# Xharlie/pointnerf

Hardware: AMD Instinct MI355X
Metric: rays/sec (render+bwd) NeRF-synth lego 800^2, K=8, 128 samp/ray (higher is better)
Workload: dtype f32 in / out / accumulate; forward GEMM operands as 2 x f16 planes (22-bit) on the f16 MFMA, 3 products per multiply-add; input-gradient GEMMs: f16 leading product + e4m3 cross terms (csrc/mixq.h), 2 product equivalents; weight-gradient GEMM operands as one f16 plane each

## Files before the change

pointnerf_amd/csrc/aggregate.hip:

```cpp
#include "mixq.h"
#include <stdlib.h>

extern "C" int pnerf_mlp_layout(int feat_dim, int64_t *offsets) {
    if (feat_dim != PN_F || !offsets) return PNERF_E_UNSUP;
    const int64_t o[PNERF_MLP_NTENSORS + 1] = {PO_W1, PO_B1, PO_W2, PO_B2, PO_W3, PO_B3, PO_W4, PO_B4, PO_W5, PO_B5,
                                               PO_WC1, PO_BC1, PO_WC2, PO_BC2, PO_WC3, PO_BC3, PO_WC4, PO_BC4, PO_TOTAL};
    for (int i = 0; i <= PNERF_MLP_NTENSORS; ++i) offsets[i] = o[i];
    return 0;
}
extern "C" size_t pnerf_mlp_packed_bytes(void) { return (size_t)PKC_END; }

namespace {
struct PackHDesc { int src, ld, trans, Mreal, Kreal, NCH, MB, dst, cm1, ck1; };
__device__ __forceinline__ float pn_pack_scale(const char *packed, int cm1, int ck1, int m, int k) {
    float f = 1.f;
    if (cm1 && m < (cm1 - 1 < PN_CS_C1 ? PN_H : PN_HC)) f = pn_col_scale(packed, cm1 - 1)[m];
    if (ck1) f *= pn_col_scale_inv(packed, ck1 - 1)[k];
    return f;
}
struct ColScaleDesc { int first, units, n_cons; struct { int src, ld, rows; } cons[2]; };
struct ColScaleTable { ColScaleDesc d[7]; };
__global__ __launch_bounds__(256) void k_pack_colscale(ColScaleTable t, const float *__restrict__ params, char *__restrict__ packed) {
    __shared__ unsigned red[256];
    const ColScaleDesc d = t.d[blockIdx.x];
// ... 48 lines not shown
    pn_mode_saturate();
    const PackMDesc d = t.d[blockIdx.y];
    auto W = [&](int m, int k) -> float {
        return (m < d.Mreal && k < d.Kreal) ? (d.trans ? params[d.src + k * d.ld + m] * pn_pack_scale(packed, d.cm1, d.ck1, m, k) : params[d.src + m * d.ld + k]) : 0.f;
    };
    uint4 *img = reinterpret_cast<uint4 *>(packed + d.dst);
    unsigned *sc = reinterpret_cast<unsigned *>(img + PN_MIMG_U4(d.NT, d.MB));
    const int nsup = PN_MIX_NS * d.MB * 64, ntail = d.NT * d.MB * 64;
    for (int e = blockIdx.x * 256 + threadIdx.x; e < nsup + ntail; e += gridDim.x * 256) {
        if (e < nsup) {
            const int lane = e & 63, mb = (e >> 6) % d.MB, s = (e >> 6) / d.MB, m = 32 * mb + (lane & 31), hf = lane >> 5;
            uint4 *o = img + ((size_t)(s * d.MB + mb) * 8) * 64 + lane;
#pragma unroll
            for (int r = 0; r < 4; ++r) {
                const int k0 = 64 * s + 16 * r + 8 * hf;
                unsigned h[4], lo[4];
#pragma unroll
                for (int j = 0; j < 4; ++j) pn_split2_rne(W(m, k0 + 2 * j), W(m, k0 + 2 * j + 1), h[j], lo[j]);
                o[r * 64] = make_uint4(h[0], h[1], h[2], h[3]);
            }
            unsigned scw = 0u;
#pragma unroll
            for (int j = 0; j < 2; ++j) {
                float wh[16], wm[16], mx = 0.f;
#pragma unroll
                for (int i = 0; i < 32; ++i) {
                    const float w = W(m, 64 * s + 32 * j + i);
#ifdef PN_EMU
                    const float wc = fmaxf(fminf(w, 65504.f), -65504.f);
#else
                    const float wc = w;
#endif
                    const float h = (float)(_Float16)wc;
                    mx = fmaxf(mx, fmaxf(fabsf(h), fabsf(w - h) * 2048.f));
                }
#pragma unroll
                for (int i = 0; i < 16; ++i) {
                    const float w = W(m, 8 * (8 * s + 4 * j + 2 * hf + (i >> 3)) + (i & 7));
#ifdef PN_EMU
                    const float wc = fmaxf(fminf(w, 65504.f), -65504.f);
#else
                    const float wc = w;
#endif
                    wh[i] = (float)(_Float16)wc; wm[i] = w - wh[i];
                }
                int ex = 0;
                const float fr = frexpf(mx, &ex);
                int be = mx > 0.f ? (fr > 0.875f ? ex - 8 : ex - 9) : 0;
                be = be < -100 ? -100 : (be > 100 ? 100 : be);
                const float sh = __uint_as_float((unsigned)(be + 127) << 23), sm = __uint_as_float((unsigned)(be + 127 - 11) << 23);
                scw |= (unsigned)(be + 127) << (8 * j);
#pragma unroll
                for (int tt = 0; tt < 2; ++tt) {
                    unsigned q[4];
#pragma unroll
                    for (int w4 = 0; w4 < 4; ++w4) {
                        const float *src = (w4 < 2 ? wm : wh) + 8 * tt + 4 * (w4 & 1);
                        const float scl = w4 < 2 ? sm : sh;
                        pn_s2 r = {0, 0};
                        r = __builtin_amdgcn_cvt_scalef32_pk_fp8_f32(r, src[0], src[1], scl, false);
                        r = __builtin_amdgcn_cvt_scalef32_pk_fp8_f32(r, src[2], src[3], scl, true);
                        q[w4] = __builtin_bit_cast(unsigned, r);
                    }
                    o[(4 + 2 * j + tt) * 64] = make_uint4(q[0], q[1], q[2], q[3]);
                }
            }
            sc[(size_t)(s * d.MB + mb) * 64 + lane] = scw;
        } else {
            const int e2 = e - nsup, lane = e2 & 63, mb = (e2 >> 6) % d.MB, tc = (e2 >> 6) / d.MB, m = 32 * mb + (lane & 31);
            const int k0 = 256 + 16 * tc + 8 * (lane >> 5);
            unsigned h[4], lo[4];
#pragma unroll
            for (int j = 0; j < 4; ++j) pn_split2_sat(W(m, k0 + 2 * j), W(m, k0 + 2 * j + 1), h[j], lo[j]);
            uint4 *o = img + (size_t)PN_MIX_NS * d.MB * 8 * 64 + ((size_t)(tc * d.MB + mb) * 2) * 64 + lane;
            o[0] = make_uint4(h[0], h[1], h[2], h[3]);
            o[64] = make_uint4(lo[0], lo[1], lo[2], lo[3]);
        }
    }
}
}

extern "C" int pnerf_mlp_pack(const float *d_params, void *d_packed, void *stream) {
    if (!d_params || !d_packed) return PNERF_E_INVAL;
    PackHTable th = {{
        {PO_W1, PN_IN1, 0, PN_H, PN_IN1, 18, 8, PKH_F1},
        {PO_W2, PN_H, 0, PN_H, PN_H, 16, 8, PKH_F2},
        {PO_W3, PN_IN3, 0, PN_H, PN_IN3, 17, 8, PKH_F3},
        {PO_W4, PN_H, 0, PN_H, PN_H, 16, 8, PKH_F4},
        {PO_W4, PN_H, 1, PN_H, PN_H, 16, 8, PKH_D4, PN_CS_L3 + 1, PN_CS_L4 + 1},
        {PO_W3, PN_IN3, 1, PN_IN3, PN_H, 16, 9, PKH_D3, PN_CS_L2 + 1, PN_CS_L3 + 1},
        {PO_W2, PN_H, 1, PN_H, PN_H, 16, 8, PKH_D2, PN_CS_L1 + 1, PN_CS_L2 + 1},
        {PO_W1, PN_IN1, 1, 32 * PN_MB_D1, PN_H, 16, PN_MB_D1, PKH_D1, 0, PN_CS_L1 + 1},
        {PO_WC1, PN_INC, 0, PN_HC, PN_INC, 18, 4, PKH_FC1},
        {PO_WC2, PN_HC, 0, PN_HC, PN_HC, 8, 4, PKH_FC2},
        {PO_WC3, PN_HC, 0, PN_HC, PN_HC, 8, 4, PKH_FC3},
        {PO_WC3, PN_HC, 1, PN_HC, PN_HC, 8, 4, PKH_DC3, PN_CS_C2 + 1, PN_CS_C3 + 1},
        {PO_WC2, PN_HC, 1, PN_HC, PN_HC, 8, 4, PKH_DC2, PN_CS_C1 + 1, PN_CS_C2 + 1},
        {PO_WC1, PN_INC, 1, PN_H, PN_HC, 8, 8, PKH_DC1, PN_CS_L4 + 1, PN_CS_C1 + 1},
        {PO_W1 + 32 * PN_MB_D1, PN_IN1, 1, PN_IN1 - 32 * PN_MB_D1, PN_H, 16, 2, PKH_D1T, 0, PN_CS_L1 + 1},
    }};
    const ColScaleTable tc = {{
        {PN_CS_L1, PN_H, 1, {{PO_W2, PN_H, PN_H}}},
        {PN_CS_L2, PN_H, 1, {{PO_W3, PN_IN3, PN_H}}},
        {PN_CS_L3, PN_H, 1, {{PO_W4, PN_H, PN_H}}},
        {PN_CS_L4, PN_H, 2, {{PO_W5, PN_H, 1}, {PO_WC1, PN_INC, PN_HC}}},
        {PN_CS_C1, PN_HC, 1, {{PO_WC2, PN_HC, PN_HC}}},
        {PN_CS_C2, PN_HC, 1, {{PO_WC3, PN_HC, PN_HC}}},
        {PN_CS_C3, PN_HC, 1, {{PO_WC4, PN_HC, 3}}},
    }};
    PnProfScope prof(PNK_PACK, (hipStream_t)stream);
    hipLaunchKernelGGL(k_pack_colscale, dim3(7), dim3(256), 0, (hipStream_t)stream, tc, d_params, (char *)d_packed);
    hipLaunchKernelGGL(k_pack_h, dim3(40, 15), dim3(256), 0, (hipStream_t)stream, th, d_params, (char *)d_packed);
    PackMTable tm = {{
        {PO_W1, PN_IN1, 0, PN_H, PN_IN1, 2, 8, PKM_F1},
        {PO_W2, PN_H, 0, PN_H, PN_H, 0, 8, PKM_F2},
        {PO_W3, PN_IN3, 0, PN_H, PN_IN3, 1, 8, PKM_F3},
        {PO_W4, PN_H, 0, PN_H, PN_H, 0, 8, PKM_F4},
        {PO_W4, PN_H, 1, PN_H, PN_H, 0, 8, PKM_D4, PN_CS_L3 + 1, PN_CS_L4 + 1},
        {PO_W3, PN_IN3, 1, PN_IN3, PN_H, 0, 9, PKM_D3, PN_CS_L2 + 1, PN_CS_L3 + 1},
        {PO_W2, PN_H, 1, PN_H, PN_H, 0, 8, PKM_D2, PN_CS_L1 + 1, PN_CS_L2 + 1},
        {PO_W1, PN_IN1, 1, 32 * PN_MB_D1, PN_H, 0, PN_MB_D1, PKM_D1, 0, PN_CS_L1 + 1},
        {PO_W1 + 32 * PN_MB_D1, PN_IN1, 1, PN_IN1 - 32 * PN_MB_D1, PN_H, 0, 2, PKM_D1T, 0, PN_CS_L1 + 1},
    }};
    hipLaunchKernelGGL(k_pack_mix, dim3(12, 9), dim3(256), 0, (hipStream_t)stream, tm, d_params, (char *)d_packed);
    PN_CHECK_LAUNCH();
    return 0;
}

namespace {
template <int NT>
__global__ __launch_bounds__(256) void k_debug_mix_gemm(const float *__restrict__ x, const char *__restrict__ img, float *__restrict__ out) {
    extern __shared__ __attribute__((aligned(16))) char smem_d[];
    pn_mode_saturate();
    constexpr int K = 256 + 16 * NT;
    char *X = smem_d;
    const int tid = threadIdx.x, lane = tid & 63, wave = __builtin_amdgcn_readfirstlane(tid >> 6);
    for (int e = tid; e < PN_TILE * (K / 4); e += 256) {
        const int row = e / (K / 4), col = 4 * (e % (K / 4));
        const float4 v = *reinterpret_cast<const float4 *>(x + row * K + col);
        if (col < 256) pn_xq_store4(X, row, col, v.x, v.y, v.z, v.w);
        else pn_xt_store4(X, row, col, v.x, v.y, v.z, v.w);
    }
    __syncthreads();
    f32x16 acc[2][2];
    pn_acc_zero(acc);
    pn_gemm_mix<PN_MIX_NS, NT, 8, 2>(X, img, 2 * wave, lane, acc);
#pragma unroll
    for (int fb = 0; fb < 2; ++fb)
#pragma unroll
        for (int rb = 0; rb < 2; ++rb)
#pragma unroll
            for (int g = 0; g < 4; ++g)
#pragma unroll
                for (int i = 0; i < 4; ++i) out[(32 * rb + (lane & 31)) * PN_H + pn_d_feat(2 * wave + fb, g, lane) + i] = acc[fb][rb][4 * g + i];
}
}

extern "C" int pnerf_debug_mix_gemm(const float *d_w, int K, const float *d_x, void *d_img, float *d_out, void *stream) {
    if (!d_w || !d_x || !d_img || !d_out || (K != 256 && K != 272 && K != 288)) return PNERF_E_INVAL;
    hipStream_t s = (hipStream_t)stream;
    const int NT = (K - 256) / 16;
    PackMTable tm = {{{0, K, 0, PN_H, K, NT, 8, 0}}};
    hipLaunchKernelGGL(k_pack_mix, dim3(12, 1), dim3(256), 0, s, tm, d_w, (char *)d_img);
    const void *fn = NT == 0 ? (const void *)k_debug_mix_gemm<0> : NT == 1 ? (const void *)k_debug_mix_gemm<1> : (const void *)k_debug_mix_gemm<2>;
    if (hipFuncSetAttribute(fn, hipFuncAttributeMaxDynamicSharedMemorySize, PN_XBYTES) != hipSuccess) return PNERF_E_LAUNCH;
    if (NT == 0) hipLaunchKernelGGL(k_debug_mix_gemm<0>, dim3(1), dim3(256), PN_XBYTES, s, d_x, (const char *)d_img, d_out);
    else if (NT == 1) hipLaunchKernelGGL(k_debug_mix_gemm<1>, dim3(1), dim3(256), PN_XBYTES, s, d_x, (const char *)d_img, d_out);
    else hipLaunchKernelGGL(k_debug_mix_gemm<2>, dim3(1), dim3(256), PN_XBYTES, s, d_x, (const char *)d_img, d_out);
    PN_CHECK_LAUNCH();
    return 0;
}

namespace {
__global__ __launch_bounds__(64) void k_debug_mfma_f16(const uint4 *__restrict__ a, const uint4 *__restrict__ b, float *__restrict__ d) {
    f32x16 acc;
#pragma unroll
    for (int r = 0; r < 16; ++r) acc[r] = 0.f;
    acc = __builtin_amdgcn_mfma_f32_32x32x16_f16(__builtin_bit_cast(pn_h8, a[threadIdx.x]), __builtin_bit_cast(pn_h8, b[threadIdx.x]), acc, 0, 0, 0);
#pragma unroll
    for (int r = 0; r < 16; ++r) d[threadIdx.x * 16 + r] = acc[r];
}
}
namespace {
__global__ __launch_bounds__(256) void k_debug_split(const float *__restrict__ x, long long n, unsigned *__restrict__ h, unsigned *__restrict__ m, int sat) {
    for (long long i = (long long)blockIdx.x * 256 + threadIdx.x; 2 * i < n; i += (long long)gridDim.x * 256) {
        unsigned hh, mm;
        if (sat) pn_split2_sat(x[2 * i], x[2 * i + 1], hh, mm);
        else pn_split2(x[2 * i], x[2 * i + 1], hh, mm);
        h[i] = hh; m[i] = mm;
    }
}
}
extern "C" int pnerf_debug_split(const float *d_x, int64_t n, void *d_h, void *d_m, int sat, void *stream) {
    if (!d_x || !d_h || !d_m || n < 0 || (n & 1)) return PNERF_E_INVAL;
    if (n == 0) return 0;
    hipLaunchKernelGGL(k_debug_split, dim3(64), dim3(256), 0, (hipStream_t)stream, d_x, (long long)n, (unsigned *)d_h, (unsigned *)d_m, sat);
    PN_CHECK_LAUNCH();
    return 0;
}

namespace {
template <int NF> __global__ __launch_bounds__(256) void k_debug_pe(const float *__restrict__ x, long long n, float *__restrict__ out) {
    for (long long i = (long long)blockIdx.x * 256 + threadIdx.x; i < n; i += (long long)gridDim.x * 256) {
        float s[NF], c[NF];
        pn_pe_octaves<NF>(x[i], s, c);
#pragma unroll
        for (int f = 0; f < NF; ++f) { out[(i * NF + f) * 2] = s[f]; out[(i * NF + f) * 2 + 1] = c[f]; }
    }
}
}
extern "C" int pnerf_debug_pe(const float *d_x, int64_t n, int nfreq, float *d_out, void *stream) {
    if (!d_x || !d_out || n < 0 || nfreq < 1 || nfreq > 5) return PNERF_E_INVAL;
    if (n == 0) return 0;
    hipStream_t s = (hipStream_t)stream;
    switch (nfreq) {
        case 1: hipLaunchKernelGGL(k_debug_pe<1>, dim3(64), dim3(256), 0, s, d_x, (long long)n, d_out); break;
        case 2: hipLaunchKernelGGL(k_debug_pe<2>, dim3(64), dim3(256), 0, s, d_x, (long long)n, d_out); break;
        case 3: hipLaunchKernelGGL(k_debug_pe<3>, dim3(64), dim3(256), 0, s, d_x, (long long)n, d_out); break;
        case 4: hipLaunchKernelGGL(k_debug_pe<4>, dim3(64), dim3(256), 0, s, d_x, (long long)n, d_out); break;
        default: hipLaunchKernelGGL(k_debug_pe<5>, dim3(64), dim3(256), 0, s, d_x, (long long)n, d_out); break;
    }
    PN_CHECK_LAUNCH();
    return 0;
}

extern "C" int pnerf_debug_mfma_f16(const void *d_a, const void *d_b, float *d_out, void *stream) {
    if (!d_a || !d_b || !d_out) return PNERF_E_INVAL;
    hipLaunchKernelGGL(k_debug_mfma_f16, dim3(1), dim3(64), 0, (hipStream_t)stream, (const uint4 *)d_a, (const uint4 *)d_b, d_out);
    PN_CHECK_LAUNCH();
    return 0;
}

size_t pn_saved_walk(void *base, long long n_valid, int K, PnSaved &s) {
    const int TS = pn_tile_samples(K);
    const long long tiles = (n_valid + TS - 1) / TS + 2 * PN_NCLS + 1;
    s.rows = tiles * PN_TILE;
    s.samples = ((tiles * TS + PN_CTILE - 1) / PN_CTILE + 1) * PN_CTILE;
    PnCarver cv(base);
    const size_t rg = (size_t)s.rows / 8, rgc = (size_t)s.samples / 8;
    auto planes = [&](uint4 *&x0, uint4 *&h2, uint4 *&h1, uint4 *&h3, uint4 *&dy1, uint4 *&dy2, uint4 *&dy3, uint4 *&dy4) {
        x0 = cv.take<uint4>(rg * PN_NF1); h2 = cv.take<uint4>(rg * PN_NF1);
        h1 = cv.take<uint4>(rg * PN_H); h3 = cv.take<uint4>(rg * PN_H);
        dy1 = cv.take<uint4>(rg * PN_H); dy2 = cv.take<uint4>(rg * PN_H);
        dy3 = cv.take<uint4>(rg * PN_H); dy4 = cv.take<uint4>(rg * PN_H);
    };
    auto cplanes = [&](uint4 *&xc, uint4 *&c1, uint4 *&c2, uint4 *&dc1, uint4 *&dc2, uint4 *&dc3) {
        xc = cv.take<uint4>(rgc * PN_NF1); c1 = cv.take<uint4>(rgc * PN_HC); c2 = cv.take<uint4>(rgc * PN_HC);
        dc1 = cv.take<uint4>(rgc * PN_HC); dc2 = cv.take<uint4>(rgc * PN_HC); dc3 = cv.take<uint4>(rgc * PN_HC);
    };
    planes(s.x0k, s.h2k, s.h1k, s.h3k, s.dy1k, s.dy2k, s.dy3k, s.dy4k);
    s.h4r = cv.take<uint4>((size_t)s.rows * 32 * 2);
    s.arow = cv.take<float>((size_t)s.rows); s.rmeta = cv.take<int4>((size_t)s.rows);
    s.lmask = cv.take<unsigned>((size_t)tiles * 3 * 512);
    s.gscale = cv.take<unsigned>(PN_GS_WORDS);
    s.fs = cv.take<float>((size_t)s.samples * PN_H); s.dfs = cv.take<float>((size_t)s.samples * PN_H);
    s.c3 = cv.take<float>((size_t)s.samples * PN_HC);
    cplanes(s.xck, s.c1k, s.c2k, s.dc1k, s.dc2k, s.dc3k);
    s.cmask = cv.take<unsigned>((size_t)s.samples / PN_CTILE * 2 * 256);
    s.wg2 = pn_arith().wgrad_planes == 2 ? 1 : 0;
    s.x0m = s.h1m = s.h2m = s.h3m = s.dy1m = s.dy2m = s.dy3m = s.dy4m = nullptr;
    s.xcm = s.c1m = s.c2m = s.dc1m = s.dc2m = s.dc3m = nullptr;
    if (s.wg2) {
        planes(s.x0m, s.h2m, s.h1m, s.h3m, s.dy1m, s.dy2m, s.dy3m, s.dy4m);
        cplanes(s.xcm, s.c1m, s.c2m, s.dc1m, s.dc2m, s.dc3m);
    }
    pn_cls_walk(cv, s);
    return cv.off;
}
void pn_cls_walk(PnCarver &cv, PnSaved &s) {
    s.cls_list = cv.take<int>((size_t)s.samples);
    s.cls_info = cv.take<int>(PN_CI_WORDS);
    s.cls_tmp = cv.take<int>((size_t)2 * s.samples + pn_scan_scratch_ints(s.samples) + 8);
}
size_t pn_saved_bytes(long long n_valid, int K) { PnSaved s; return pn_saved_walk(nullptr, n_valid, K, s); }
PnSaved pn_saved_carve(void *base, long long n_valid, int K) { PnSaved s; pn_saved_walk(base, n_valid, K, s); return s; }

extern "C" size_t pnerf_agg_saved_bytes(int64_t n_valid_samples, int K) {
    if (K <= 0 || K > PNERF_MAX_K || n_valid_samples < 0) return 0;
    return pn_saved_bytes(n_valid_samples, K);
}

namespace {
struct FwdArgs {
    pnerf_camera cam;
    const float *xyz, *emb, *conf, *dir, *color;
    const float *params;
    const float4 *packed;
    const float *raydir, *sample_loc;
    const float *xyz_pers, *loc_pers;
    const int *pidx, *valid_list, *counters;
    const int *cls_list, *cls_info;
    int cls, Kstride;
    int save_x0;
    int R, SR, K, TS;
    long long cap_samples;
    float *decoded, *weight;
    PnSaved sv;
};
struct FwdArgsF : FwdArgs { const float *frames; };
template <bool FRAMES> struct FwdArgsOf { using type = FwdArgs; };
template <> struct FwdArgsOf<true> { using type = FwdArgsF; };

namespace {
struct ClsArgs { const int *valid_list, *counters, *pidx; int K, n, ncls; int kc[PN_NCLS], ts[PN_NCLS]; };

__global__ void k_cls_flags(ClsArgs c, int which, int *__restrict__ flags) {
    const int vs = blockIdx.x * blockDim.x + threadIdx.x;
    if (vs >= c.n) return;
    const int Ns = c.counters[0] < c.n ? c.counters[0] : c.n;
    int f = 0;
    if (vs < Ns) {
        const long long si = c.valid_list[vs];
        int hv = 0;
        for (int k = 0; k < c.K; ++k)
            if (c.pidx[si * c.K + k] >= 0) hv = k + 1;
        int cl = 0;
        for (int j = 1; j < c.ncls; ++j)
            if (hv <= c.kc[j]) cl = j;
        f = cl == which;
    }
    flags[vs] = f;
}

__global__ void k_cls_gather(ClsArgs c, int which, const int *__restrict__ pos, const int *__restrict__ count, int *__restrict__ cls_list,
                             int *__restrict__ info) {
    const int n = *count, base = info[PN_CI_VBASE + which];
    for (int i = blockIdx.x * blockDim.x + threadIdx.x; i < n; i += gridDim.x * blockDim.x) cls_list[base + i] = c.valid_list[pos[i]];
    if (blockIdx.x == 0 && threadIdx.x == 0) {
        const int tiles = (n + c.ts[which] - 1) / c.ts[which], tb = info[PN_CI_TBASE + which];
        info[PN_CI_COUNT + which] = n;
        if (which + 1 < PN_NCLS) { info[PN_CI_VBASE + which + 1] = base + n; info[PN_CI_TBASE + which + 1] = tb + tiles + 1; }
        info[PN_CI_TILES] = tb + tiles + 1;
    }
}

__global__ void k_cls_zero_gaps(PnSaved sv, int ncls, int save_x0) {
    const int c = blockIdx.y;
    if (c >= ncls) return;
    if ((blockIdx.x == 0 && !save_x0) || (blockIdx.x == 8 && save_x0)) return;
    const long long gap = (c + 1 < PN_NCLS ? sv.cls_info[PN_CI_TBASE + c + 1] : sv.cls_info[PN_CI_TILES]) - 1;
    uint4 *arrs[9] = {sv.x0k, sv.h2k, sv.h1k, sv.h3k, sv.dy1k, sv.dy2k, sv.dy3k, sv.dy4k, sv.x0k};
    uint4 *arrm[9] = {sv.x0m, sv.h2m, sv.h1m, sv.h3m, sv.dy1m, sv.dy2m, sv.dy3m, sv.dy4m, nullptr};
    const int which = blockIdx.x;
    const int nf = which == 8 ? 64 : which < 2 ? PN_NF1 : PN_H;
    uint4 *p = arrs[which] + gap * 8 * nf;
    for (int i = threadIdx.x; i < 8 * nf; i += blockDim.x) p[i] = make_uint4(0u, 0u, 0u, 0u);
    if (sv.wg2 && arrm[which]) {
        uint4 *pm = arrm[which] + gap * 8 * nf;
        for (int i = threadIdx.x; i < 8 * nf; i += blockDim.x) pm[i] = make_uint4(0u, 0u, 0u, 0u);
    }
}
}

}

int pn_class_slots(int K, int kc[PN_NCLS]) {
    if (K % 4 == 0) { kc[0] = K; kc[1] = K / 2; kc[2] = K / 4; return 3; }
    kc[0] = K; kc[1] = kc[2] = 0;
    return 1;
}

int pn_classify(const PnSaved &sv, const int32_t *d_valid_list, const int32_t *d_counters, const int32_t *d_pidx, int K, long long n_valid,
                bool train, bool save_x0, hipStream_t s) {
    ClsArgs c;
    c.valid_list = d_valid_list; c.counters = d_counters; c.pidx = d_pidx; c.K = K; c.n = (int)n_valid;
    c.ncls = pn_class_slots(K, c.kc);
    for (int j = 0; j < PN_NCLS; ++j) c.ts[j] = c.kc[j] > 0 ? pn_tile_samples(c.kc[j]) : 1;
    if (hipMemsetAsync(sv.cls_info, 0, PN_CI_WORDS * sizeof(int), s) != hipSuccess) return PNERF_E_LAUNCH;
    if (n_valid <= 0) return 0;
    int *flags = sv.cls_tmp, *pos = flags + n_valid, *cnt = pos + n_valid, *scratch = cnt + 8;
    PnProfScope prof(PNK_COMPACT, s);
    for (int j = 0; j < c.ncls; ++j) {
        hipLaunchKernelGGL(k_cls_flags, dim3(pn_cdiv(n_valid, 256)), dim3(256), 0, s, c, j, flags);
        int rc = pn_compact_gt0_i32(flags, n_valid, pos, cnt, scratch, s);
        if (rc) return rc;
        hipLaunchKernelGGL(k_cls_gather, dim3(256), dim3(256), 0, s, c, j, pos, cnt, sv.cls_list, sv.cls_info);
    }
    if (train) hipLaunchKernelGGL(k_cls_zero_gaps, dim3(9, c.ncls), dim3(256), 0, s, sv, c.ncls, save_x0 ? 1 : 0);
    PN_CHECK_LAUNCH();
    return 0;
}


namespace {

constexpr int FL_EX = PN_XBYTES, FL_W5 = FL_EX + PN_TILE * 8 * 4, FL_ROW = FL_W5 + PN_H * 4, FL_CLAIM = FL_ROW + 4 * PN_TILE * 4 , FL_BYTES = FL_CLAIM + 16;
static_assert(2 * FL_BYTES <= 160 * 1024, "two forward workgroups must fit the 160 KB LDS");

struct FGather {
    float4 e0, e1;
    float px, py, pz, lx, ly, lz, cf;
    float ppx, ppy, ppz, lpx, lpy, lpz;
    float dxv, dyv, dzv, cx, cy, cz, rx, ry, rz;
    float fx, fy, fz, gx, gy, gz;
};

__device__ __forceinline__ int f_sample_of(const FwdArgs &a, long long tile, int row, int Ns, unsigned kinv) {
    const int ls = pn_row_div(row, kinv);
    const long long vs = tile * a.TS + ls;
    return (ls < a.TS && vs < Ns) ? a.valid_list[vs] : -1;
}

template <bool PERS, bool FRAMES = false>
__device__ __forceinline__ void f_gather(const FwdArgs &a, FGather &G, int si_, int p_, int q, const float *frames = nullptr) {
    const int p = p_ > 0 ? p_ : 0, si = si_ > 0 ? si_ : 0;
    const float *ep = a.emb + (long long)p * PN_F + PN_EPT * q;
    G.e0 = *reinterpret_cast<const float4 *>(ep); G.e1 = *reinterpret_cast<const float4 *>(ep + 4);
    G.px = a.xyz[3 * p]; G.py = a.xyz[3 * p + 1]; G.pz = a.xyz[3 * p + 2];
    G.lx = a.sample_loc[(long long)si * 3]; G.ly = a.sample_loc[(long long)si * 3 + 1]; G.lz = a.sample_loc[(long long)si * 3 + 2];
    if (PERS) {
        G.ppx = a.xyz_pers[3 * p]; G.ppy = a.xyz_pers[3 * p + 1]; G.ppz = a.xyz_pers[3 * p + 2];
        G.lpx = a.loc_pers[(long long)si * 3]; G.lpy = a.loc_pers[(long long)si * 3 + 1]; G.lpz = a.loc_pers[(long long)si * 3 + 2];
    }
    G.cf = a.conf[p];
    if (FRAMES) {
        const int r = si / a.SR, fr = q < 3 ? q : 2;
        const int ps_ = a.pidx[(long long)si * a.Kstride], ps = ps_ > 0 ? ps_ : 0;
        const float *fp = frames + (long long)p * 9 + 3 * fr, *gp = frames + (long long)ps * 9 + 3 * fr;
        G.fx = fp[0]; G.fy = fp[1]; G.fz = fp[2];
        G.gx = gp[0]; G.gy = gp[1]; G.gz = gp[2];
        G.dxv = a.dir[3 * p]; G.dyv = a.dir[3 * p + 1]; G.dzv = a.dir[3 * p + 2];
        G.rx = a.raydir[3 * r]; G.ry = a.raydir[3 * r + 1]; G.rz = a.raydir[3 * r + 2];
        if (q == 0) { G.cx = a.color[3 * p]; G.cy = a.color[3 * p + 1]; G.cz = a.color[3 * p + 2]; }
    } else if (q == 0) {
        const int r = si / a.SR;
        G.dxv = a.dir[3 * p]; G.dyv = a.dir[3 * p + 1]; G.dzv = a.dir[3 * p + 2];
        G.cx = a.color[3 * p]; G.cy = a.color[3 * p + 1]; G.cz = a.color[3 * p + 2];
        G.rx = a.raydir[3 * r]; G.ry = a.raydir[3 * r + 1]; G.rz = a.raydir[3 * r + 2];
    }
}

template <bool PERS, bool MIX = false, bool FRAMES = false>
__device__ __forceinline__ void f_build(const FwdArgs &a, const FGather &G, char *X, float *exb, float *wraw, int *sidx, int si, int p, int row, int q) {
    const float dwx = G.px - G.lx, dwy = G.py - G.ly, dwz = G.pz - G.lz;
    float ppx, ppy, pcz, spx, spy, scz;
    if (PERS) {
        ppx = G.ppx; ppy = G.ppy; pcz = G.ppz; spx = G.lpx; spy = G.lpy; scz = G.lpz;
    } else {
        float pcx, pcy, scx, scy;
        if (FRAMES) {
            const float *M = a.cam.camrot;
            const float x = G.px - a.cam.campos[0], y = G.py - a.cam.campos[1], z = G.pz - a.cam.campos[2];
            const float u = G.lx - a.cam.campos[0], v = G.ly - a.cam.campos[1], w = G.lz - a.cam.campos[2];
            pcx = __builtin_fmaf(z, M[6], __builtin_fmaf(y, M[3], x * M[0]));
            pcy = __builtin_fmaf(z, M[7], __builtin_fmaf(y, M[4], x * M[1]));
            pcz = __builtin_fmaf(z, M[8], __builtin_fmaf(y, M[5], x * M[2]));
            scx = __builtin_fmaf(w, M[6], __builtin_fmaf(u, M[0], v * M[3]));
            scy = __builtin_fmaf(w, M[7], __builtin_fmaf(u, M[1], v * M[4]));
            scz = __builtin_fmaf(w, M[8], __builtin_fmaf(u, M[2], v * M[5]));
        } else {
        rot3(a.cam.camrot, G.px - a.cam.campos[0], G.py - a.cam.campos[1], G.pz - a.cam.campos[2], false, pcx, pcy, pcz);
        rot3(a.cam.camrot, G.lx - a.cam.campos[0], G.ly - a.cam.campos[1], G.lz - a.cam.campos[2], false, scx, scy, scz);
        }
        ppx = pcx / pcz; ppy = pcy / pcz; spx = scx / scz; spy = scy / scz;
    }
    float d0, d1, d2;
    if (FRAMES) d0 = d1 = d2 = dwx * G.fx + dwy * G.fy + dwz * G.fz;
    else rot3(a.cam.rw2c, dwx, dwy, dwz, true, d0, d1, d2);
    const float d3 = ppx * pcz - spx * scz, d4 = ppy * pcz - spy * scz, d5 = pcz - scz;
    const float da = q == 0 ? d0 : q == 1 ? d1 : q == 2 ? d2 : d3;
    const float db = q == 0 ? d4 : d5;
    const float e[8] = {G.e0.x, G.e0.y, G.e0.z, G.e0.w, G.e1.x, G.e1.y, G.e1.z, G.e1.w};
    if (MIX) {
        pn_xq_store4(X, row, PN_EPT * q, e[0], e[1], e[2], e[3]);
        pn_xq_store4(X, row, PN_EPT * q + 4, e[4], e[5], e[6], e[7]);
#pragma unroll
        for (int i = 0; i < 8; i += 2) {
            const int col = PN_F + (PN_EPT * q + i) * 6;
            float s0[3], c0[3], s1[3], c1[3];
            pn_pe_octaves<3>(e[i], s0, c0);
            pn_pe_octaves<3>(e[i + 1], s1, c1);
            pn_xq_store4(X, row, col, s0[0], c0[0], s0[1], c0[1]);
            pn_xq_store4(X, row, col + 4, s0[2], c0[2], s1[0], c1[0]);
            pn_xq_store4(X, row, col + 8, s1[1], c1[1], s1[2], c1[2]);
        }
    } else {
    pn_xt_store4(X, row, PN_EPT * q, e[0], e[1], e[2], e[3]); pn_xt_store4(X, row, PN_EPT * q + 4, e[4], e[5], e[6], e[7]);
#pragma unroll
    for (int i = 0; i < 8; ++i) {
        const int dd = PN_EPT * q + i;
        float s[3], c[3];
        pn_pe_octaves<3>(e[i], s, c);
        pn_xt_store2(X, row, PN_F + dd * 6, s[0], c[0]);
        pn_xt_store2(X, row, PN_F + dd * 6 + 2, s[1], c[1]);
        pn_xt_store2(X, row, PN_F + dd * 6 + 4, s[2], c[2]);
    }
    }
#pragma unroll
    for (int j = 0; j < 2; ++j) {
        const int comp = q + 4 * j;
        if (comp < 6) {
            float s[5], c[5];
            pn_pe_octaves<5>(j == 0 ? da : db, s, c);
#pragma unroll
            for (int f = 0; f < 5; ++f) {
                if (MIX) pn_xa_store2(X, row, PN_F * 7 + (comp * 5 + f) * 2, s[f], c[f]);
                else pn_xt_store2(X, row, PN_F * 7 + (comp * 5 + f) * 2, s[f], c[f]);
            }
        }
    }
    if (q == 3) pn_xt_store4(X, row, PN_ONES1, 1.f, 0.f, 0.f, 0.f);
    float fvx = 0.f, fvy = 0.f, fvz = 0.f, fqx = 0.f, fqy = 0.f, fqz = 0.f;
    if (FRAMES) {
        fvx = G.rx * G.gx + G.ry * G.gy + G.rz * G.gz;
        fqx = G.dxv * G.fx + G.dyv * G.fy + G.dzv * G.fz;
        fvy = __shfl_down(fvx, 1, 64); fvz = __shfl_down(fvx, 2, 64);
        fqy = __shfl_down(fqx, 1, 64); fqz = __shfl_down(fqx, 2, 64);
    }
    if (q == 0) {
        float vx, vy, vz, qx, qy, qz;
        if (FRAMES) { vx = fvx; vy = fvy; vz = fvz; qx = fqx; qy = fqy; qz = fqz; }
        else {
        rot3(a.cam.rw2c, G.rx, G.ry, G.rz, true, vx, vy, vz);
        rot3(a.cam.rw2c, G.dxv, G.dyv, G.dzv, true, qx, qy, qz);
        }
        float *ex = exb + row * 8;
        *reinterpret_cast<float4 *>(ex) = make_float4(G.cx, G.cy, G.cz, qx - vx);
        if (FRAMES) {
            *reinterpret_cast<float4 *>(ex + 4) = make_float4(qy - vy, qz - vz, __builtin_fmaf(qz, vz, __builtin_fmaf(qx, vx, qy * vy)), 1.f);
            wraw[row] = p >= 0 ? 1.0f / fmaxf(sqrtf(__builtin_fmaf(dwz, dwz, __builtin_fmaf(dwx, dwx, dwy * dwy))), 1e-6f) : 0.f;
        } else {
        *reinterpret_cast<float4 *>(ex + 4) = make_float4(qy - vy, qz - vz, qx * vx + qy * vy + qz * vz, 1.f);
        wraw[row] = p >= 0 ? 1.0f / fmaxf(sqrtf(dwx * dwx + dwy * dwy + dwz * dwz), 1e-6f) : 0.f;
        }
        sidx[row] = si;
    }
}

__device__ __forceinline__ void f_acc_bias(const float *__restrict__ bias, int wave, int lane, f32x16 (&acc)[PN_NFB][2]) {
#pragma unroll
    for (int fb = 0; fb < PN_NFB; ++fb)
#pragma unroll
        for (int g = 0; g < 4; ++g) {
            const float4 b = *reinterpret_cast<const float4 *>(bias + pn_d_feat(PN_NFB * wave + fb, g, lane));
#pragma unroll
            for (int rb = 0; rb < 2; ++rb) { acc[fb][rb][4 * g] = b.x; acc[fb][rb][4 * g + 1] = b.y; acc[fb][rb][4 * g + 2] = b.z; acc[fb][rb][4 * g + 3] = b.w; }
        }
}
template <bool BITS, bool MIX = false, bool HR = false>
__device__ __forceinline__ void f_epilogue(const f32x16 (&acc)[PN_NFB][2], char *X, int wave, int lane, unsigned (&mw)[PN_NFB]) {
#pragma unroll
    for (int fb = 0; fb < PN_NFB; ++fb) mw[fb] = 0u;
#pragma unroll
    for (int fb = 0; fb < PN_NFB; ++fb)
#pragma unroll
        for (int rb = 0; rb < 2; ++rb)
#pragma unroll
            for (int g = 0; g < 4; ++g) {
                const int f0 = pn_d_feat(PN_NFB * wave + fb, g, lane);
                float v[4] = {acc[fb][rb][4 * g], acc[fb][rb][4 * g + 1], acc[fb][rb][4 * g + 2], acc[fb][rb][4 * g + 3]};
                if (BITS) {
#pragma unroll
                    for (int i = 0; i < 4; ++i) mw[fb] = __builtin_amdgcn_alignbit(mw[fb], __float_as_uint(v[i]), 31);
                }
#pragma unroll
                for (int i = 0; i < 4; ++i) v[i] = fmaxf(v[i], 0.01f * v[i]);
                if (MIX) pn_xq_store4(X, 32 * rb + (lane & 31), f0, v[0], v[1], v[2], v[3]);
                else if (HR) pn_xt_store4(X, 32 * rb + (lane & 31), f0, v[0], v[1], v[2], v[3]);
                else pn_x_store4<false>(X, 32 * rb + (lane & 31), f0, v[0], v[1], v[2], v[3]);
            }
}
__device__ __forceinline__ void f_store_masks(unsigned *__restrict__ lmask, long long gtile, int layer, int wave, int lane, const unsigned (&mw)[PN_NFB]) {
#pragma unroll
    for (int fb = 0; fb < PN_NFB; ++fb) lmask[((gtile * 3 + layer) * 8 + PN_NFB * wave + fb) * 64 + lane] = mw[fb];
}

template <int KC, bool TRAIN>
__device__ __forceinline__ void f_tail(const FwdArgs &a, const char *X, const float *w5s, const float *wrow, const int *sidx, float b5,
                                       long long tile, long long gtile, int tid, float *wraw = nullptr) {
    constexpr int NS = KC == 0 ? 1 : 8 / (KC == 0 ? 1 : KC);
    const int lane = tid & 63, cg = tid & 31, r0 = 8 * (tid >> 5);
    const float4 wa = *reinterpret_cast<const float4 *>(w5s + 8 * cg), wb = *reinterpret_cast<const float4 *>(w5s + 8 * cg + 4);
    float pa[8];
    float4 fa[NS], fb[NS];
#pragma unroll
    for (int j = 0; j < NS; ++j) fa[j] = fb[j] = make_float4(0.f, 0.f, 0.f, 0.f);
#pragma unroll
    for (int i = 0; i < 8; ++i) {
        const int r = r0 + i;
        const uint4 h = *reinterpret_cast<const uint4 *>(X + r * PN_XRS + cg * 16);
        const uint4 m = *reinterpret_cast<const uint4 *>(X + PN_XPLANE + r * PN_XRS + cg * 16);
        if (TRAIN) {
            pn_f4 th = {__uint_as_float(h.x), __uint_as_float(h.y), __uint_as_float(h.z), __uint_as_float(h.w)};
            pn_f4 tm = {__uint_as_float(m.x), __uint_as_float(m.y), __uint_as_float(m.z), __uint_as_float(m.w)};
            PN_STREAM_STORE(th, reinterpret_cast<pn_f4 *>(a.sv.h4r + (gtile * PN_TILE + r) * 32 + cg));
            PN_STREAM_STORE(tm, reinterpret_cast<pn_f4 *>(a.sv.h4r + (a.sv.rows + gtile * PN_TILE + r) * 32 + cg));
        }
        float s = 0.f;
        s = pn_fma2_lo(h.x, m.x, wa.x, s); s = pn_fma2_hi(h.x, m.x, wa.y, s); s = pn_fma2_lo(h.y, m.y, wa.z, s); s = pn_fma2_hi(h.y, m.y, wa.w, s);
        s = pn_fma2_lo(h.z, m.z, wb.x, s); s = pn_fma2_hi(h.z, m.z, wb.y, s); s = pn_fma2_lo(h.w, m.w, wb.z, s); s = pn_fma2_hi(h.w, m.w, wb.w, s);
        pa[i] = s;
        if (KC != 0) {
            const float w = wrow[r];
            float4 &f0 = fa[i / (KC == 0 ? 1 : KC)], &f1 = fb[i / (KC == 0 ? 1 : KC)];
            f0.x = pn_fma2_lo(h.x, m.x, w, f0.x); f0.y = pn_fma2_hi(h.x, m.x, w, f0.y); f0.z = pn_fma2_lo(h.y, m.y, w, f0.z); f0.w = pn_fma2_hi(h.y, m.y, w, f0.w);
            f1.x = pn_fma2_lo(h.z, m.z, w, f1.x); f1.y = pn_fma2_hi(h.z, m.z, w, f1.y); f1.z = pn_fma2_lo(h.w, m.w, w, f1.z); f1.w = pn_fma2_hi(h.w, m.w, w, f1.w);
        }
    }
#pragma unroll
    for (int j = 0; j < (KC == 0 ? 0 : NS); ++j) {
        const long long vs = tile * (PN_TILE / (KC == 0 ? 1 : KC)) + (r0 / (KC == 0 ? 1 : KC)) + j;
        if (vs < a.cap_samples) {
            *reinterpret_cast<float4 *>(a.sv.fs + vs * PN_H + 8 * cg) = fa[j];
            *reinterpret_cast<float4 *>(a.sv.fs + vs * PN_H + 8 * cg + 4) = fb[j];
        }
    }
    {
        const bool b4 = lane & 16, b3 = lane & 8, b2 = lane & 4;
#pragma unroll
        for (int j = 0; j < 4; ++j) { const float send = b4 ? pa[j] : pa[j + 4], keep = b4 ? pa[j + 4] : pa[j]; pa[j] = keep + __shfl_xor(send, 16, 64); }
#pragma unroll
        for (int j = 0; j < 2; ++j) { const float send = b3 ? pa[j] : pa[j + 2], keep = b3 ? pa[j + 2] : pa[j]; pa[j] = keep + __shfl_xor(send, 8, 64); }
        { const float send = b2 ? pa[0] : pa[1], keep = b2 ? pa[1] : pa[0]; pa[0] = keep + __shfl_xor(send, 4, 64); }
        pa[0] += __shfl_xor(pa[0], 2, 64);
        pa[0] += __shfl_xor(pa[0], 1, 64);
        const int i = ((lane >> 4) & 1) * 4 + ((lane >> 3) & 1) * 2 + ((lane >> 2) & 1), r = r0 + i;
        const float x = pa[0] + b5 - 1.0f;
        float sg = pn_softplus(x) * wrow[r];
        if (TRAIN && (lane & 3) == 0) a.sv.arow[gtile * PN_TILE + r] = x;
        if (KC == 0) {
            if ((lane & 3) == 0) wraw[r] = sg;
            return;
        }
        if (KC >= 2) sg += __shfl_xor(sg, 4, 64);
        if (KC >= 4) sg += __shfl_xor(sg, 8, 64);
        if (KC >= 8) sg += __shfl_xor(sg, 16, 64);
        if ((lane & 3) == 0 && (i % (KC == 0 ? 1 : KC)) == 0) {
            const int si = sidx[r];
            if (si >= 0) a.decoded[(long long)si * 4] = sg;
        }
    }
}

#ifdef PN_PHASE_TRACE
PN_TR_DECL(pn_trace_fwd);
PN_TR_SPAN_DECL(pn_span_fwd);
#endif
template <bool TRAIN, bool PERS, int NP, bool WG2 = false, bool FRAMES = false>
__global__ __launch_bounds__(PN_NTHR, PN_NW / 2) void k_agg_forward(typename FwdArgsOf<FRAMES>::type a) {
    constexpr bool MIX = NP == 4;
    static_assert(!FRAMES || (!TRAIN && NP == 3), "per-point frames: the default inference arithmetic only");
    constexpr bool HR = !MIX;
    constexpr bool HC = TRAIN && !WG2;
    static_assert(!(MIX && WG2), "the two-plane weight-gradient mode keeps f16x3.h's arithmetic everywhere");
    pn_mode_saturate();
    extern __shared__ __attribute__((aligned(16))) char smem_f[];
    char *X = smem_f;
    float *exb = reinterpret_cast<float *>(smem_f + FL_EX), *w5s = reinterpret_cast<float *>(smem_f + FL_W5);
    float *wraw = reinterpret_cast<float *>(smem_f + FL_ROW), *wrow = wraw + PN_TILE, *wnrm = wrow + PN_TILE;
    int *sidx = reinterpret_cast<int *>(wnrm + PN_TILE);
    const float *frames = nullptr;
    if constexpr (FRAMES) frames = a.frames;
    const int tid0 = threadIdx.x;
    const int K = a.K, TS = a.TS;
    const unsigned kinv = pn_kinv(K);
    const int Ns = a.cls_info[PN_CI_COUNT + a.cls];
    const long long vb = a.cls_info[PN_CI_VBASE + a.cls], tb = a.cls_info[PN_CI_TBASE + a.cls];
    a.valid_list = a.cls_list + vb; a.cap_samples = Ns;
    a.sv.fs += vb * PN_H;
    const long long ntiles = ((long long)Ns + TS - 1) / TS;
    const float *P = a.params;
    const char *img = reinterpret_cast<const char *>(a.packed);
    if (tid0 < PN_H) w5s[tid0] = P[PO_W5 + tid0];
    const float b5 = P[PO_B5];
    const int tile_last = (int)ntiles, grid = gridDim.x;
    int t0 = blockIdx.x, t1 = t0 + grid, t2 = t1 + grid;
    if (t0 >= tile_last) return;
    int *claim_ctr = a.sv.cls_info + PN_CI_CLAIM + a.cls, *claim_w = reinterpret_cast<int *>(smem_f + FL_CLAIM);
    int nclaim = 0;

    long long tile = t0;
    int si0, si1, si2, p0, p1;
    FGather G;
    {
        const int row = tid0 / PN_TPR, q = tid0 % PN_TPR, k = row - pn_row_div(row, kinv) * K;
        si0 = f_sample_of(a, tile, row, Ns, kinv); si1 = t1 < tile_last ? f_sample_of(a, t1, row, Ns, kinv) : -1;
        si2 = t2 < tile_last ? f_sample_of(a, t2, row, Ns, kinv) : -1;
        p0 = si0 >= 0 ? a.pidx[(long long)si0 * a.Kstride + k] : -1;
        p1 = si1 >= 0 ? a.pidx[(long long)si1 * a.Kstride + k] : -1;
        f_gather<PERS, FRAMES>(a, G, si0, p0, q, frames);
// ... 398 lines not shown
```

pointnerf_amd/csrc/pn_common.h:

```cpp
#pragma once
#include <hip/hip_runtime.h>
#include <stdint.h>
#include <stddef.h>
#include "pnerf.h"

#define PN_WAVE 64

#define PN_CHECK_LAUNCH()                                         \
    do {                                                          \
        if (hipGetLastError() != hipSuccess) return PNERF_E_LAUNCH; \
    } while (0)

static inline size_t pn_align(size_t x, size_t a = 256) { return (x + a - 1) / a * a; }
static inline int pn_cdiv(long long a, long long b) { return (int)((a + b - 1) / b); }

static inline int pn_capped_grid(long long tiles, long long cap) { return (int)(tiles < cap ? (tiles > 0 ? tiles : 1) : cap); }
static inline int pn_cu_count() {
    int dev = 0, ncu = 256;
    if (hipGetDevice(&dev) != hipSuccess) return 0;
    return hipDeviceGetAttribute(&ncu, hipDeviceAttributeMultiprocessorCount, dev) == hipSuccess ? ncu : 256;
}

struct PnCarver {
    char *base; size_t off;
    explicit PnCarver(void *p) : base((char *)p), off(0) {}
    template <class T> T *take(size_t n) {
        T *r = base ? (T *)(base + off) : nullptr;
        off += pn_align(n * sizeof(T));
        return r;
    }
};

enum PnKernelId { PNK_GRID = 0, PNK_PROBE, PNK_NEIGHBORS, PNK_COMPACT, PNK_PACK, PNK_AGG_FWD, PNK_COLOR_FWD, PNK_RAYMARCH_FWD,
                  PNK_RAYMARCH_BWD, PNK_COLOR_BWD, PNK_AGG_BWD, PNK_WGRAD, PNK_WGRAD_REDUCE, PNK_GATHER, PNK_ADAM, PNK_COUNT };
extern int pn_prof_enabled;
void pn_prof_mark(int id, bool begin, hipStream_t s);
struct PnProfScope {
    int id; hipStream_t s;
    PnProfScope(int id_, hipStream_t s_) : id(id_), s(s_) { if (pn_prof_enabled) pn_prof_mark(id, true, s); }
    ~PnProfScope() { if (pn_prof_enabled) pn_prof_mark(id, false, s); }
};

size_t pn_scan_scratch_ints(long long n);
int pn_exclusive_scan_i32(const int *in, int *out, long long n, int *scratch, hipStream_t s);
int pn_compact_gt0_i32(const int *in, long long n, int *list, int *count_out, int *scratch, hipStream_t s);

__device__ __forceinline__ int pn_zero_one_point(int p, int n) { return p < 0 ? 0 : (p >= n ? n - 1 : p); }
struct PnZeroOne {
    float c, eps;
    __device__ __forceinline__ PnZeroOne(float conf, float eps_) : c(fminf(fmaxf(conf, 1e-4f), 1.0f)), eps(eps_) {}
    __device__ __forceinline__ bool inside() const { return c >= eps && c <= 1.f - eps; }
    __device__ __forceinline__ float value() const {
        const float v = fminf(fmaxf(c, eps), 1.f - eps);
        return logf(v) + logf(1.f - v);
    }
    __device__ __forceinline__ float grad(float gs) const { return inside() ? gs * (1.f / c - 1.f / (1.f - c)) : 0.f; }
};

struct PnGridDev {
    float ox, oy, oz;
    float vx, vy, vz;
    int gx, gy, gz;
    int by, bz;
    int P;
    const char *base;
    const int *info;
    const uint4 *bricks;
    const uint32_t *occ;
    const float4 *pts;
};

struct PnGridLayout {
    size_t info, bricks, occ, pts, ostart, keys, cnt, tmp_idx, ocell, bocc, bpts, brank, bbase, scan, total;
    long long G, NB;
};
PnGridLayout pn_grid_layout(const pnerf_grid_params *gp, int n);
PnGridDev pn_grid_dev(const pnerf_grid_params *gp, const void *ws, int n_unused);

__device__ __forceinline__ int pn_cell(float p, float o, float v) {
    return (int)floorf((p - o) / v);
}
__host__ __device__ __forceinline__ int pn_brick_of(int x, int y, int z, int by, int bz) { return ((x >> 2) * by + (y >> 2)) * bz + (z >> 2); }
__host__ __device__ __forceinline__ int pn_cell_in_brick(int x, int y, int z) { return ((x & 3) << 4) | ((y & 3) << 2) | (z & 3); }
__device__ __forceinline__ const int *pn_grid_ostart(const PnGridDev &g) { return (const int *)(g.base + (size_t)g.info[PNERF_GI_OSTART_OFF] * 256); }
__device__ __forceinline__ int pn_cell_points(const PnGridDev &g, const int *__restrict__ ostart, int cell0, int x, int y, int z, int &st) {
    const int brick = pn_brick_of(x, y, z, g.by, g.bz), local = pn_cell_in_brick(x, y, z);
    const uint4 rec = g.bricks[brick];
    const unsigned long long bits = ((unsigned long long)rec.y << 32) | rec.x;
    if (!((bits >> local) & 1ull) || brick * 64 + local == cell0) return 0;
    const int o = (int)rec.z + __popcll(bits & ((1ull << local) - 1ull));
    st = ostart[o];
    return min(g.P, ostart[o + 1] - st);
}
```

pointnerf_amd/csrc/scan.hip:

```cpp
#include "pn_common.h"

namespace {
constexpr int TPB = 256;
constexpr int EPT = 8;
constexpr int CHUNK = TPB * EPT;

template <int MODE> __device__ __forceinline__ int xf(int v) { return MODE == 0 ? v : (v > 0 ? 1 : 0); }

__device__ __forceinline__ int block_excl_scan(int v, int *block_total, int *lds4) {
    const int lane = threadIdx.x & 63, wave = threadIdx.x >> 6;
    int x = v;
#pragma unroll
    for (int off = 1; off < 64; off <<= 1) {
        int y = __shfl_up(x, off, 64);
        if (lane >= off) x += y;
    }
    if (lane == 63) lds4[wave] = x;
    __syncthreads();
    int woff = 0, tot = 0;
#pragma unroll
    for (int w = 0; w < TPB / 64; ++w) {
        int t = lds4[w];
        if (w < wave) woff += t;
        tot += t;
    }
    *block_total = tot;
    __syncthreads();
    return woff + x - v;
}

template <int MODE>
__global__ __launch_bounds__(TPB) void k_scan_reduce(const int *__restrict__ in, long long n, int *__restrict__ bsum) {
    __shared__ int lds4[4];
    long long base = (long long)blockIdx.x * CHUNK + (long long)threadIdx.x * EPT;
    int s = 0;
#pragma unroll
    for (int e = 0; e < EPT; ++e) {
        long long i = base + e;
        if (i < n) s += xf<MODE>(in[i]);
    }
    int tot;
    block_excl_scan(s, &tot, lds4);
    if (threadIdx.x == 0) bsum[blockIdx.x] = tot;
}

__global__ __launch_bounds__(TPB) void k_scan_bsums(int *bsum, int nb) {
    __shared__ int lds4[4];
    int carry = 0;
    for (int base = 0; base < nb; base += TPB) {
        int i = base + threadIdx.x;
        int v = i < nb ? bsum[i] : 0;
        int tot;
        int ex = block_excl_scan(v, &tot, lds4);
        if (i < nb) bsum[i] = carry + ex;
        carry += tot;
    }
    if (threadIdx.x == 0) bsum[nb] = carry;
}

template <int MODE>
__global__ __launch_bounds__(TPB) void k_scan_apply(const int *__restrict__ in, long long n, const int *__restrict__ bsum,
                                                    int nb, int *__restrict__ out, int *__restrict__ count) {
    __shared__ int lds4[4];
    long long base = (long long)blockIdx.x * CHUNK + (long long)threadIdx.x * EPT;
    int v[EPT];
    int s = 0;
#pragma unroll
    for (int e = 0; e < EPT; ++e) {
        long long i = base + e;
        v[e] = i < n ? xf<MODE>(in[i]) : 0;
        s += v[e];
    }
    int tot;
    int ex = block_excl_scan(s, &tot, lds4) + bsum[blockIdx.x];
#pragma unroll
    for (int e = 0; e < EPT; ++e) {
        long long i = base + e;
        if (i < n) {
            if (MODE == 0) out[i] = ex;
            else if (v[e]) out[ex] = (int)i;
        }
        ex += v[e];
    }
    if (blockIdx.x == 0 && threadIdx.x == 0) {
        if (MODE == 0) out[n] = bsum[nb];
        else *count = bsum[nb];
    }
}
}

size_t pn_scan_scratch_ints(long long n) { return (size_t)pn_cdiv(n > 0 ? n : 1, CHUNK) + 2; }

int pn_exclusive_scan_i32(const int *in, int *out, long long n, int *scratch, hipStream_t s) {
    int nb = pn_cdiv(n > 0 ? n : 1, CHUNK);
    hipLaunchKernelGGL(k_scan_reduce<0>, dim3(nb), dim3(TPB), 0, s, in, n, scratch);
    hipLaunchKernelGGL(k_scan_bsums, dim3(1), dim3(TPB), 0, s, scratch, nb);
    hipLaunchKernelGGL(k_scan_apply<0>, dim3(nb), dim3(TPB), 0, s, in, n, scratch, nb, out, (int *)nullptr);
    PN_CHECK_LAUNCH();
    return 0;
}

int pn_compact_gt0_i32(const int *in, long long n, int *list, int *count_out, int *scratch, hipStream_t s) {
    int nb = pn_cdiv(n > 0 ? n : 1, CHUNK);
    hipLaunchKernelGGL(k_scan_reduce<1>, dim3(nb), dim3(TPB), 0, s, in, n, scratch);
    hipLaunchKernelGGL(k_scan_bsums, dim3(1), dim3(TPB), 0, s, scratch, nb);
    hipLaunchKernelGGL(k_scan_apply<1>, dim3(nb), dim3(TPB), 0, s, in, n, scratch, nb, list, count_out);
    PN_CHECK_LAUNCH();
    return 0;
}
```

Baseline: 2.193 million.

## Replace per-class compaction loop with single multi-way count/scan/scatter partition

Sample classification previously ran flag, three-kernel compaction and gather once per class (up to 3 classes, so about 15 launches) and re-read pidx each time. Now one count kernel computes each sample's class once, with int4-vectorised pidx reads, and records per-block tallies via wave ballots. A row-wise scan over the tallies follows, then a scatter kernel writes each sample into its class segment and fills the info table. This cuts launches and redundant global reads. The cost is a single-block-per-row scan over the block tallies, and the new layout requires the tally scratch to fit in cls_tmp.

New measurement: 2.201 million, median of 6. Within noise of the previous version (+0.3%).

```diff
diff --git a/pointnerf_amd/csrc/aggregate.hip b/pointnerf_amd/csrc/aggregate.hip
--- a/pointnerf_amd/csrc/aggregate.hip
+++ b/pointnerf_amd/csrc/aggregate.hip
@@ -374,35 +374,75 @@
 template <> struct FwdArgsOf<true> { using type = FwdArgsF; };
 
 namespace {
-struct ClsArgs { const int *valid_list, *counters, *pidx; int K, n, ncls; int kc[PN_NCLS], ts[PN_NCLS]; };
-
-__global__ void k_cls_flags(ClsArgs c, int which, int *__restrict__ flags) {
-    const int vs = blockIdx.x * blockDim.x + threadIdx.x;
-    if (vs >= c.n) return;
+struct ClsArgs { const int *valid_list, *counters, *pidx; int K, n, ncls; int kc[PN_NCLS], ts[PN_NCLS]; int vec4 ; };
+
+constexpr int CLS_TPB = 256;
+
+__global__ __launch_bounds__(CLS_TPB) void k_cls_count(ClsArgs c, int *__restrict__ cls_of, int *__restrict__ tally, int nb) {
+    __shared__ int wcnt[PN_NCLS][CLS_TPB / 64];
+    const int vs = blockIdx.x * CLS_TPB + threadIdx.x, lane = threadIdx.x & 63, wave = threadIdx.x >> 6;
     const int Ns = c.counters[0] < c.n ? c.counters[0] : c.n;
-    int f = 0;
+    int cl = -1;
     if (vs < Ns) {
         const long long si = c.valid_list[vs];
         int hv = 0;
-        for (int k = 0; k < c.K; ++k)
-            if (c.pidx[si * c.K + k] >= 0) hv = k + 1;
-        int cl = 0;
+        if (c.vec4) {
+            const int4 *p = reinterpret_cast<const int4 *>(c.pidx + si * c.K);
+            for (int k = 0; k < c.K; k += 4) {
+                const int4 v = p[k >> 2];
+                if (v.x >= 0) hv = k + 1;
+                if (v.y >= 0) hv = k + 2;
+                if (v.z >= 0) hv = k + 3;
+                if (v.w >= 0) hv = k + 4;
+            }
+        } else {
+            for (int k = 0; k < c.K; ++k)
+                if (c.pidx[si * c.K + k] >= 0) hv = k + 1;
+        }
+        cl = 0;
         for (int j = 1; j < c.ncls; ++j)
             if (hv <= c.kc[j]) cl = j;
-        f = cl == which;
-    }
-    flags[vs] = f;
-}
-
-__global__ void k_cls_gather(ClsArgs c, int which, const int *__restrict__ pos, const int *__restrict__ count, int *__restrict__ cls_list,
-                             int *__restrict__ info) {
-    const int n = *count, base = info[PN_CI_VBASE + which];
-    for (int i = blockIdx.x * blockDim.x + threadIdx.x; i < n; i += gridDim.x * blockDim.x) cls_list[base + i] = c.valid_list[pos[i]];
+    }
+    if (vs < c.n) cls_of[vs] = cl;
+    for (int j = 0; j < c.ncls; ++j) {
+        const int cnt = __popcll(__ballot(cl == j));
+        if (lane == 0) wcnt[j][wave] = cnt;
+    }
+    __syncthreads();
+    if ((int)threadIdx.x < c.ncls) {
+        int t = 0;
+        for (int w = 0; w < CLS_TPB / 64; ++w) t += wcnt[threadIdx.x][w];
+        tally[(size_t)threadIdx.x * (nb + 1) + blockIdx.x] = t;
+    }
+}
+
+__global__ __launch_bounds__(CLS_TPB) void k_cls_scatter(ClsArgs c, const int *__restrict__ cls_of, const int *__restrict__ tally, int nb,
+                                                         int *__restrict__ cls_list, int *__restrict__ info) {
+    __shared__ int wcnt[PN_NCLS][CLS_TPB / 64];
+    const int vs = blockIdx.x * CLS_TPB + threadIdx.x, lane = threadIdx.x & 63, wave = threadIdx.x >> 6;
+    const int cl = vs < c.n ? cls_of[vs] : -1;
+    int rank = 0;
+    for (int j = 0; j < c.ncls; ++j) {
+        const unsigned long long m = __ballot(cl == j);
+        if (lane == 0) wcnt[j][wave] = __popcll(m);
+        if (cl == j) rank = __popcll(m & ((1ull << lane) - 1ull));
+    }
+    __syncthreads();
+    if (cl >= 0) {
+        int pos = tally[(size_t)cl * (nb + 1) + blockIdx.x] + rank;
+        for (int w = 0; w < wave; ++w) pos += wcnt[cl][w];
+        for (int j = 0; j < cl; ++j) pos += tally[(size_t)j * (nb + 1) + nb];
+        cls_list[pos] = c.valid_list[vs];
+    }
     if (blockIdx.x == 0 && threadIdx.x == 0) {
-        const int tiles = (n + c.ts[which] - 1) / c.ts[which], tb = info[PN_CI_TBASE + which];
-        info[PN_CI_COUNT + which] = n;
-        if (which + 1 < PN_NCLS) { info[PN_CI_VBASE + which + 1] = base + n; info[PN_CI_TBASE + which + 1] = tb + tiles + 1; }
-        info[PN_CI_TILES] = tb + tiles + 1;
+        int base = 0, tb = 0;
+        for (int j = 0; j < c.ncls; ++j) {
+            const int n = tally[(size_t)j * (nb + 1) + nb], tiles = (n + c.ts[j] - 1) / c.ts[j];
+            info[PN_CI_COUNT + j] = n;
+            base += n; tb += tiles + 1;
+            if (j + 1 < PN_NCLS) { info[PN_CI_VBASE + j + 1] = base; info[PN_CI_TBASE + j + 1] = tb; }
+            info[PN_CI_TILES] = tb;
+        }
     }
 }
 
@@ -437,17 +477,17 @@
     ClsArgs c;
     c.valid_list = d_valid_list; c.counters = d_counters; c.pidx = d_pidx; c.K = K; c.n = (int)n_valid;
     c.ncls = pn_class_slots(K, c.kc);
+    c.vec4 = K % 4 == 0 && (reinterpret_cast<uintptr_t>(d_pidx) & 15) == 0;
     for (int j = 0; j < PN_NCLS; ++j) c.ts[j] = c.kc[j] > 0 ? pn_tile_samples(c.kc[j]) : 1;
     if (hipMemsetAsync(sv.cls_info, 0, PN_CI_WORDS * sizeof(int), s) != hipSuccess) return PNERF_E_LAUNCH;
     if (n_valid <= 0) return 0;
-    int *flags = sv.cls_tmp, *pos = flags + n_valid, *cnt = pos + n_valid, *scratch = cnt + 8;
+    const int nb = pn_cdiv(n_valid, CLS_TPB);
+    int *cls_of = sv.cls_tmp, *tally = cls_of + n_valid;
     PnProfScope prof(PNK_COMPACT, s);
-    for (int j = 0; j < c.ncls; ++j) {
-        hipLaunchKernelGGL(k_cls_flags, dim3(pn_cdiv(n_valid, 256)), dim3(256), 0, s, c, j, flags);
-        int rc = pn_compact_gt0_i32(flags, n_valid, pos, cnt, scratch, s);
-        if (rc) return rc;
-        hipLaunchKernelGGL(k_cls_gather, dim3(256), dim3(256), 0, s, c, j, pos, cnt, sv.cls_list, sv.cls_info);
-    }
+    hipLaunchKernelGGL(k_cls_count, dim3(nb), dim3(CLS_TPB), 0, s, c, cls_of, tally, nb);
+    int rc = pn_exclusive_scan_rows_i32(tally, c.ncls, nb, s);
+    if (rc) return rc;
+    hipLaunchKernelGGL(k_cls_scatter, dim3(nb), dim3(CLS_TPB), 0, s, c, cls_of, tally, nb, sv.cls_list, sv.cls_info);
     if (train) hipLaunchKernelGGL(k_cls_zero_gaps, dim3(9, c.ncls), dim3(256), 0, s, sv, c.ncls, save_x0 ? 1 : 0);
     PN_CHECK_LAUNCH();
     return 0;
diff --git a/pointnerf_amd/csrc/pn_common.h b/pointnerf_amd/csrc/pn_common.h
--- a/pointnerf_amd/csrc/pn_common.h
+++ b/pointnerf_amd/csrc/pn_common.h
@@ -44,6 +44,7 @@
 size_t pn_scan_scratch_ints(long long n);
 int pn_exclusive_scan_i32(const int *in, int *out, long long n, int *scratch, hipStream_t s);
 int pn_compact_gt0_i32(const int *in, long long n, int *list, int *count_out, int *scratch, hipStream_t s);
+int pn_exclusive_scan_rows_i32(int *rows, int nrows, int nb, hipStream_t s);
 
 __device__ __forceinline__ int pn_zero_one_point(int p, int n) { return p < 0 ? 0 : (p >= n ? n - 1 : p); }
 struct PnZeroOne {
diff --git a/pointnerf_amd/csrc/scan.hip b/pointnerf_amd/csrc/scan.hip
--- a/pointnerf_amd/csrc/scan.hip
+++ b/pointnerf_amd/csrc/scan.hip
@@ -58,6 +58,21 @@
     if (threadIdx.x == 0) bsum[nb] = carry;
 }
 
+__global__ __launch_bounds__(TPB) void k_scan_rows(int *rows, int nb) {
+    __shared__ int lds4[4];
+    int *row = rows + (size_t)blockIdx.x * (nb + 1);
+    int carry = 0;
+    for (int base = 0; base < nb; base += TPB) {
+        int i = base + threadIdx.x;
+        int v = i < nb ? row[i] : 0;
+        int tot;
+        int ex = block_excl_scan(v, &tot, lds4);
+        if (i < nb) row[i] = carry + ex;
+        carry += tot;
+    }
+    if (threadIdx.x == 0) row[nb] = carry;
+}
+
 template <int MODE>
 __global__ __launch_bounds__(TPB) void k_scan_apply(const int *__restrict__ in, long long n, const int *__restrict__ bsum,
                                                     int nb, int *__restrict__ out, int *__restrict__ count) {
@@ -100,6 +115,12 @@
     return 0;
 }
 
+int pn_exclusive_scan_rows_i32(int *rows, int nrows, int nb, hipStream_t s) {
+    hipLaunchKernelGGL(k_scan_rows, dim3(nrows), dim3(TPB), 0, s, rows, nb);
+    PN_CHECK_LAUNCH();
+    return 0;
+}
+
 int pn_compact_gt0_i32(const int *in, long long n, int *list, int *count_out, int *scratch, hipStream_t s) {
     int nb = pn_cdiv(n > 0 ? n : 1, CHUNK);
     hipLaunchKernelGGL(k_scan_reduce<1>, dim3(nb), dim3(TPB), 0, s, in, n, scratch);
```
